# rasd3/3D-Dual-Fusion

Measured on AMD Instinct MI355X. Metric: nuScenes sweeps/sec (0.075 m voxel, ~60k pts), higher is better.
Workload: dtype f32 (fp32-grade throughout: every matrix-core GEMM -- C>=32 sparse convs, neck / head convs, FFN, query linears, image projection, value GEMM -- takes its fp32 operands as fp16 hi+lo pairs, 22 significand bits, 3 MFMA products, fp32 accumulate: <= 4e-6 of scale against float64, the grade of the exac

## Files before the change

3d-dual-fusion_amd/csrc/ffn.hip:

```cpp
#include <stdlib.h>

#include <string.h>

#include "common.h"

namespace df3d {

DF3D_SPLIT_OVERFLOW_TU(ffn)

constexpr int FFN_WQ = 8 * 2 * 64;

template <int C>
__global__ __launch_bounds__(256) void pack_ffn_kernel(const float *__restrict__ w1, const float *__restrict__ w2,
                                                       int H, u32x4 *__restrict__ out) {
  constexpr int KB = C / 32, CT = C / 16, SPC = KB + 4;
  size_t i = (size_t)blockIdx.x * blockDim.x + threadIdx.x;
  size_t total = (size_t)(H / 128) * SPC * FFN_WQ;
  if (i >= total) return;
  int lane = (int)(i & 63);
  int part = (int)((i >> 6) & 1);
  int t = (int)((i >> 7) & 7);
  int sj = (int)((i >> 10) % SPC);
  int c = (int)((i >> 10) / SPC);
  int n = lane & 15, g = lane >> 4;
  float wv[8];
#pragma unroll
  for (int e = 0; e < 8; ++e) {
    float w = 0.f;
    if (sj < KB) {
      int hid = c * 128 + t * 16 + n;
      int ch = sj * 32 + g * 8 + e;
      w = w1[(size_t)hid * C + ch];
    } else if (t < CT) {
      int q = sj - KB;
      int col = n * CT + t;
      int hid = c * 128 + (2 * q + (e >> 2)) * 16 + 4 * g + (e & 3);
      w = w2[(size_t)col * H + hid];
    }
    wv[e] = w;
  }
  u32x4 o;
#pragma unroll
  for (int e = 0; e < 4; ++e) {
    unsigned hi, lo;
    split_pair_w(wv[2 * e], wv[2 * e + 1], hi, lo);
    o[e] = part ? lo : hi;
  }
  out[i] = o;
}

struct FfnArgs {
  const float *x;
  const u32x4 *w;
  const float *b1, *b2;
  const float *res;
  const float *ln_g, *ln_b;
  float eps;
  float *out;
  long long rows;
  int H;
  int dbg;
  int bf16;
};

struct FfnJobs {
  FfnArgs s[4];
};

template <int NW, int RT, int NP = 2, int C = 128>
__global__ __launch_bounds__(NW * 64) void ffn_split_kernel(FfnJobs jobs) {
  constexpr int KB = C / 32, CT = C / 16, SPC = KB + 4;
  const FfnArgs &a = jobs.s[blockIdx.y];
  if ((long long)blockIdx.x * (16 * RT * NW) >= a.rows) return;
  constexpr int NT = NW * 64, WR = 16 * RT, TM = NW * WR;
  constexpr int WPT = FFN_WQ / NT;
  static_assert(FFN_WQ % NT == 0, "tile must divide over the workgroup");
  __shared__ u32x4 Wl[2][FFN_WQ];

  const int tid = threadIdx.x, lane = tid & 63, wave = tid >> 6;
  const int g = lane >> 4, n = lane & 15;
  const long long wrow0 = (long long)blockIdx.x * TM + wave * WR;
  const int nchunks = a.H / 128;
  const int steps = nchunks * SPC;

  u32x4 xh[RT][KB], xl[RT][KB];
#pragma unroll
  for (int rt = 0; rt < RT; ++rt) {
    const long long row_n = wrow0 + rt * 16 + n;
    const long long row_ld = row_n < a.rows ? row_n : a.rows - 1;
#pragma unroll
    for (int kb = 0; kb < KB; ++kb) {
      const float *p = a.x + row_ld * C + kb * 32 + g * 8;
      f32x4 v0 = *(const f32x4 *)p, v1 = *(const f32x4 *)(p + 4);
      split_pair(v0[0], v0[1], xh[rt][kb][0], xl[rt][kb][0]);
      split_pair(v0[2], v0[3], xh[rt][kb][1], xl[rt][kb][1]);
      split_pair(v1[0], v1[1], xh[rt][kb][2], xl[rt][kb][2]);
      split_pair(v1[2], v1[3], xh[rt][kb][3], xl[rt][kb][3]);
    }
  }

  static_assert(SPC % 2 == 0, "register set = step parity");
  u32x4 wreg[2][WPT];
  auto load_w = [&](int s, int set) {
    s = s < steps ? s : steps - 1;
    const u32x4 *src = a.w + (size_t)s * FFN_WQ;
#pragma unroll
    for (int i = 0; i < WPT; ++i) wreg[set][i] = src[tid + NT * i];
  };
  auto store_w = [&](int buf, int set) {
#pragma unroll
    for (int i = 0; i < WPT; ++i) Wl[buf][tid + NT * i] = wreg[set][i];
  };

  f32x4 acc2[RT][CT];
#pragma unroll
  for (int rt = 0; rt < RT; ++rt)
#pragma unroll
    for (int ct = 0; ct < CT; ++ct) acc2[rt][ct] = (f32x4){0.f, 0.f, 0.f, 0.f};

  load_w(0, 0);
  store_w(0, 0);
  load_w(1, 1);
  load_w(2, 0);
  for (int c = 0; c < nchunks; ++c) {
    f32x4 acc1[RT][8];
#pragma unroll
    for (int rt = 0; rt < RT; ++rt)
#pragma unroll
      for (int t = 0; t < 8; ++t) acc1[rt][t] = (f32x4){0.f, 0.f, 0.f, 0.f};
#pragma unroll
    for (int kb = 0; kb < KB; ++kb) {
      const int s = c * SPC + kb;
      __syncthreads();
      if (!(a.dbg & 2)) {
        store_w((s + 1) & 1, (kb + 1) & 1);
        load_w(s + 3, (kb + 1) & 1);
      }
      const u32x4 *wb = Wl[s & 1] + lane;
      if (a.dbg & 1) continue;
      u32x4 fq[2][4];
#pragma unroll
      for (int q = 0; q < 4; q += (NP == 2 ? 1 : 2)) fq[0][q] = wb[q * 64];
#pragma unroll
      for (int t = 0; t < 8; t += 2) {
        const int cur = (t >> 1) & 1;
        if (t + 2 < 8) {
#pragma unroll
          for (int q = 0; q < 4; q += (NP == 2 ? 1 : 2)) fq[cur ^ 1][q] = wb[((t + 2) * 2 + q) * 64];
        }
        const u32x4 ah0 = fq[cur][0], al0 = fq[cur][1], ah1 = fq[cur][2], al1 = fq[cur][3];
        if constexpr (NP == 2) {
#pragma unroll
          for (int rt = 0; rt < RT; ++rt) {
            acc1[rt][t] = DF3D_MFMA_F16(ah0, xl[rt][kb], acc1[rt][t]);
            acc1[rt][t + 1] = DF3D_MFMA_F16(ah1, xl[rt][kb], acc1[rt][t + 1]);
          }
#pragma unroll
          for (int rt = 0; rt < RT; ++rt) {
            acc1[rt][t] = DF3D_MFMA_F16(al0, xh[rt][kb], acc1[rt][t]);
            acc1[rt][t + 1] = DF3D_MFMA_F16(al1, xh[rt][kb], acc1[rt][t + 1]);
          }
        }
#pragma unroll
        for (int rt = 0; rt < RT; ++rt) {
          acc1[rt][t] = DF3D_MFMA_F16(ah0, xh[rt][kb], acc1[rt][t]);
          acc1[rt][t + 1] = DF3D_MFMA_F16(ah1, xh[rt][kb], acc1[rt][t + 1]);
        }
      }
    }
    u32x4 hh[RT][4], hl[RT][4];
#pragma unroll
    for (int q = 0; q < 4; ++q) {
#pragma unroll
      for (int half = 0; half < 2; ++half) {
        const int t = 2 * q + half;
        const f32x4 b = *(const f32x4 *)(a.b1 + c * 128 + t * 16 + 4 * g);
#pragma unroll
        for (int rt = 0; rt < RT; ++rt) {
          const f32x4 hv = acc1[rt][t] * DF3D_ACC_UNSCALE + b;
          split_pair_nc(fmaxf(hv[0], 0.f), fmaxf(hv[1], 0.f), hh[rt][q][half * 2], hl[rt][q][half * 2]);
          split_pair_nc(fmaxf(hv[2], 0.f), fmaxf(hv[3], 0.f), hh[rt][q][half * 2 + 1], hl[rt][q][half * 2 + 1]);
        }
      }
    }
#pragma unroll
    for (int q = 0; q < 4; ++q) {
      const int s = c * SPC + KB + q;
      __syncthreads();
      if (!(a.dbg & 2)) {
        store_w((s + 1) & 1, (KB + q + 1) & 1);
        load_w(s + 3, (KB + q + 1) & 1);
      }
      const u32x4 *wb = Wl[s & 1] + lane;
      if (a.dbg & 1) continue;
      u32x4 fq[2][4];
#pragma unroll
      for (int k = 0; k < 4; k += (NP == 2 ? 1 : 2)) fq[0][k] = wb[k * 64];
#pragma unroll
      for (int ct = 0; ct < CT; ct += 2) {
        const int cur = (ct >> 1) & 1;
        if (ct + 2 < CT) {
#pragma unroll
          for (int k = 0; k < 4; k += (NP == 2 ? 1 : 2)) fq[cur ^ 1][k] = wb[((ct + 2) * 2 + k) * 64];
        }
        const u32x4 bh0 = fq[cur][0], bl0 = fq[cur][1], bh1 = fq[cur][2], bl1 = fq[cur][3];
        if constexpr (NP == 2) {
#pragma unroll
          for (int rt = 0; rt < RT; ++rt) {
            acc2[rt][ct] = DF3D_MFMA_F16(hl[rt][q], bh0, acc2[rt][ct]);
            acc2[rt][ct + 1] = DF3D_MFMA_F16(hl[rt][q], bh1, acc2[rt][ct + 1]);
          }
#pragma unroll
          for (int rt = 0; rt < RT; ++rt) {
            acc2[rt][ct] = DF3D_MFMA_F16(hh[rt][q], bl0, acc2[rt][ct]);
            acc2[rt][ct + 1] = DF3D_MFMA_F16(hh[rt][q], bl1, acc2[rt][ct + 1]);
          }
        }
#pragma unroll
        for (int rt = 0; rt < RT; ++rt) {
          acc2[rt][ct] = DF3D_MFMA_F16(hh[rt][q], bh0, acc2[rt][ct]);
          acc2[rt][ct + 1] = DF3D_MFMA_F16(hh[rt][q], bh1, acc2[rt][ct + 1]);
        }
      }
    }
  }

  constexpr int NV = CT / 4;
  f32x4 bias[NV], gam[NV], bet[NV];
#pragma unroll
  for (int v = 0; v < NV; ++v) {
    bias[v] = *(const f32x4 *)(a.b2 + n * CT + 4 * v);
    gam[v] = (f32x4){1.f, 1.f, 1.f, 1.f};
    bet[v] = (f32x4){0.f, 0.f, 0.f, 0.f};
    if (a.ln_g) {
      gam[v] = *(const f32x4 *)(a.ln_g + n * CT + 4 * v);
      bet[v] = *(const f32x4 *)(a.ln_b + n * CT + 4 * v);
    }
  }
#pragma unroll
  for (int rt = 0; rt < RT; ++rt) {
    const long long rbase = wrow0 + rt * 16 + 4 * g;
#pragma unroll
    for (int r = 0; r < 4; ++r) {
      const long long row = rbase + r;
      const bool live = row < a.rows;
      const long long rr = live ? row : a.rows - 1;
      f32x4 val[NV];
      float s = 0.f;
#pragma unroll
      for (int v = 0; v < NV; ++v) {
        val[v] = (f32x4){acc2[rt][4 * v][r], acc2[rt][4 * v + 1][r], acc2[rt][4 * v + 2][r], acc2[rt][4 * v + 3][r]} *
                     DF3D_ACC_UNSCALE + bias[v];
        if (a.res) val[v] += *(const f32x4 *)(a.res + rr * C + n * CT + 4 * v);
        s += val[v][0] + val[v][1] + val[v][2] + val[v][3];
      }
      if (a.ln_g) {
#pragma unroll
        for (int o = 8; o >= 1; o >>= 1) s += __shfl_xor(s, o, 64);
        const float mean = s * (1.f / C);
        float ss = 0.f;
#pragma unroll
        for (int v = 0; v < NV; ++v) {
          val[v] = val[v] - mean;
          ss += val[v][0] * val[v][0] + val[v][1] * val[v][1] + val[v][2] * val[v][2] + val[v][3] * val[v][3];
        }
#pragma unroll
        for (int o = 8; o >= 1; o >>= 1) ss += __shfl_xor(ss, o, 64);
        const float rstd = rsqrtf(ss * (1.f / C) + a.eps);
#pragma unroll
        for (int v = 0; v < NV; ++v) val[v] = val[v] * rstd * gam[v] + bet[v];
      }
      if (live) {
#pragma unroll
        for (int v = 0; v < NV; ++v) *(f32x4 *)(a.out + row * C + n * CT + 4 * v) = val[v];
      }
    }
  }
}

}

using namespace df3d;

extern "C" size_t df3d_ffn_packed_bytes(int d_model, int d_ffn) {
  if ((d_model != 128 && d_model != 64) || d_ffn <= 0 || d_ffn % 128 != 0) return 0;
  return (size_t)(d_ffn / 128) * (d_model / 32 + 4) * FFN_WQ * 16;
}

extern "C" int df3d_ffn_pack(const float *w1, const float *w2, int d_model, int d_ffn, void *packed, void *stream_) {
  hipStream_t stream = (hipStream_t)stream_;
  DF3D_CHECK_ARG(w1 && w2 && packed, "ffn_pack: null argument");
  DF3D_CHECK_ARG(df3d_ffn_packed_bytes(d_model, d_ffn) != 0,
                 "ffn_pack: the fused feed-forward kernel serves d_model 64 / 128 and d_ffn %% 128 == 0 (got %d, %d)",
                 d_model, d_ffn);
  size_t total = (size_t)(d_ffn / 128) * (d_model / 32 + 4) * FFN_WQ;
  if (d_model == 128)
    hipLaunchKernelGGL(pack_ffn_kernel<128>, dim3(cdiv((long long)total, 256)), dim3(256), 0, stream, w1, w2, d_ffn,
                       (u32x4 *)packed);
  else
    hipLaunchKernelGGL(pack_ffn_kernel<64>, dim3(cdiv((long long)total, 256)), dim3(256), 0, stream, w1, w2, d_ffn,
                       (u32x4 *)packed);
  DF3D_LAUNCH_CHECK();
  return DF3D_OK;
}

static int ffn_launch(const FfnJobs &jobs, int njobs, long long max_rows, int d_model, hipStream_t stream) {
  if (d_model == 64) {
    static const int cfg64 = getenv("DF3D_FFN_CFG64") ? atoi(getenv("DF3D_FFN_CFG64")) : 0;
    if (!jobs.s[0].bf16 && cfg64 == 44) {
      hipLaunchKernelGGL((ffn_split_kernel<4, 4, 2, 64>), dim3(cdiv(max_rows, 256), njobs), dim3(256), 0, stream, jobs);
      DF3D_LAUNCH_CHECK();
      return DF3D_OK;
    }
    if (!jobs.s[0].bf16 && (cfg64 == 82 || (cfg64 == 0 && (long long)cdiv(max_rows, 256) * njobs >= 192))) {
      hipLaunchKernelGGL((ffn_split_kernel<8, 2, 2, 64>), dim3(cdiv(max_rows, 256), njobs), dim3(512), 0, stream, jobs);
      DF3D_LAUNCH_CHECK();
      return DF3D_OK;
    }
    if (jobs.s[0].bf16)
      hipLaunchKernelGGL((ffn_split_kernel<8, 1, 1, 64>), dim3(cdiv(max_rows, 128), njobs), dim3(512), 0, stream, jobs);
    else
      hipLaunchKernelGGL((ffn_split_kernel<8, 1, 2, 64>), dim3(cdiv(max_rows, 128), njobs), dim3(512), 0, stream, jobs);
    DF3D_LAUNCH_CHECK();
    return DF3D_OK;
  }
  static const int cfg_env = getenv("DF3D_FFN_CFG") ? atoi(getenv("DF3D_FFN_CFG")) : 0;
  static int ncu = 0;
  if (!ncu) {
    hipDeviceProp_t prop;
    ncu = (hipGetDeviceProperties(&prop, 0) == hipSuccess && prop.multiProcessorCount > 0) ? prop.multiProcessorCount : 256;
  }
  const long long wg82 = (long long)cdiv(max_rows, 256) * njobs;
  static const bool balance = !(getenv("DF3D_FFN_PAD") && getenv("DF3D_FFN_PAD")[0] == '0');
  const int cfg = cfg_env ? cfg_env : (wg82 >= 160 && !(balance && wg82 > ncu) ? 82 : 81);
  if (jobs.s[0].bf16) {
    if (max_rows >= 32 * 1024 && cfg != 81 + 1000)
      hipLaunchKernelGGL((ffn_split_kernel<8, 2, 1>), dim3(cdiv(max_rows, 256), njobs), dim3(512), 0, stream, jobs);
    else
      hipLaunchKernelGGL((ffn_split_kernel<8, 1, 1>), dim3(cdiv(max_rows, 128), njobs), dim3(512), 0, stream, jobs);
    DF3D_LAUNCH_CHECK();
    return DF3D_OK;
  }
  if (cfg == 44) hipLaunchKernelGGL((ffn_split_kernel<4, 4>), dim3(cdiv(max_rows, 256), njobs), dim3(256), 0, stream, jobs);
  else if (cfg == 42) hipLaunchKernelGGL((ffn_split_kernel<4, 2>), dim3(cdiv(max_rows, 128), njobs), dim3(256), 0, stream, jobs);
  else if (cfg == 82) {
    size_t pad = 0;
    if (balance && wg82 <= ncu) {
      pad = 52 * 1024;
      static bool attr = false;
      if (!attr) {
        attr = hipFuncSetAttribute((const void *)ffn_split_kernel<8, 2>, hipFuncAttributeMaxDynamicSharedMemorySize,
                                   (int)pad) == hipSuccess;
        if (!attr) pad = 0;
      }
    }
    hipLaunchKernelGGL((ffn_split_kernel<8, 2>), dim3(cdiv(max_rows, 256), njobs), dim3(512), pad, stream, jobs);
  }
  else if (cfg == 41) hipLaunchKernelGGL((ffn_split_kernel<4, 1>), dim3(cdiv(max_rows, 64), njobs), dim3(256), 0, stream, jobs);
  else hipLaunchKernelGGL((ffn_split_kernel<8, 1>), dim3(cdiv(max_rows, 128), njobs), dim3(512), 0, stream, jobs);
  DF3D_LAUNCH_CHECK();
  return DF3D_OK;
}

static int g_ffn_bf16 = 0;
extern "C" int df3d_ffn_set_precision(int bf16) {
  g_ffn_bf16 = bf16 ? 1 : 0;
  return DF3D_OK;
}

extern "C" int df3d_ffn_fused(const float *x, long long rows, int d_model, int d_ffn, const void *packed,
                              const float *b1, const float *b2, const float *residual, const float *ln_weight,
                              const float *ln_bias, float eps, float *out, void *stream_) {
  hipStream_t stream = (hipStream_t)stream_;
  DF3D_CHECK_ARG(x && packed && b1 && b2 && out, "ffn_fused: null argument");
  DF3D_CHECK_ARG(df3d_ffn_packed_bytes(d_model, d_ffn) != 0, "ffn_fused: unsupported sizes d_model=%d d_ffn=%d",
                 d_model, d_ffn);
  DF3D_CHECK_ARG((ln_weight == nullptr) == (ln_bias == nullptr), "ffn_fused: LayerNorm needs weight and bias");
  if (rows <= 0) return DF3D_OK;
  FfnJobs jobs;
  memset(&jobs, 0, sizeof(jobs));
  jobs.s[0] = {x, (const u32x4 *)packed, b1, b2, residual, ln_weight, ln_bias, eps, out, rows, d_ffn,
               getenv("DF3D_FFN_DBG") ? atoi(getenv("DF3D_FFN_DBG")) : 0, g_ffn_bf16};
  return ffn_launch(jobs, 1, rows, d_model, stream);
}

extern "C" int df3d_ffn_fused_jobs(const df3d_ffn_job *j, int njobs, int d_model, int d_ffn, void *stream_) {
  hipStream_t stream = (hipStream_t)stream_;
  DF3D_CHECK_ARG(j && njobs >= 1 && njobs <= 4, "ffn_fused_jobs: 1..4 jobs");
  DF3D_CHECK_ARG(df3d_ffn_packed_bytes(d_model, d_ffn) != 0, "ffn_fused_jobs: unsupported sizes d_model=%d d_ffn=%d",
                 d_model, d_ffn);
  FfnJobs jobs;
  memset(&jobs, 0, sizeof(jobs));
  long long max_rows = 0;
  static const int dbg = getenv("DF3D_FFN_DBG") ? atoi(getenv("DF3D_FFN_DBG")) : 0;
  for (int i = 0; i < njobs; ++i) {
    DF3D_CHECK_ARG(j[i].rows <= 0 || (j[i].x && j[i].packed && j[i].b1 && j[i].b2 && j[i].out),
                   "ffn_fused_jobs: job %d has a null argument", i);
    DF3D_CHECK_ARG((j[i].ln_weight == nullptr) == (j[i].ln_bias == nullptr),
                   "ffn_fused_jobs: LayerNorm needs weight and bias");
    jobs.s[i] = {j[i].x, (const u32x4 *)j[i].packed, j[i].b1, j[i].b2, j[i].residual, j[i].ln_weight, j[i].ln_bias,
                 j[i].eps, j[i].out, j[i].rows > 0 ? j[i].rows : 0, d_ffn, dbg, g_ffn_bf16};
    if (j[i].rows > max_rows) max_rows = j[i].rows;
  }
  if (max_rows <= 0) return DF3D_OK;
  return ffn_launch(jobs, njobs, max_rows, d_model, stream);
}
```

Baseline: 404.0.

## Restructure fused FFN into 32-wide hidden stages with lagged ReLU/split overlap

Repacks FFN weights so each pipeline stage holds a 32-wide hidden slice of both W1 and W2, and rewrites the kernel to stream these stages through dynamic LDS. For RT>=2 it uses three buffers and a one-stage lag, so the bias+ReLU+hi/lo split of the previous slice is interleaved between the current slice's first-GEMM MFMAs, with scheduling barriers pinning the placement. This targets the serial epilogue bubble between the two GEMMs and cuts hidden-activation register pressure. In exchange it costs more LDS per workgroup, which can lower occupancy. It also drops the debug flag, the LDS padding balance heuristic and the 44 configs.

```diff
diff --git a/3d-dual-fusion_amd/csrc/ffn.hip b/3d-dual-fusion_amd/csrc/ffn.hip
--- a/3d-dual-fusion_amd/csrc/ffn.hip
+++ b/3d-dual-fusion_amd/csrc/ffn.hip
@@ -2,43 +2,50 @@
 
 #include <string.h>
 
+#include <type_traits>
+
 #include "common.h"
 
 namespace df3d {
 
 DF3D_SPLIT_OVERFLOW_TU(ffn)
 
-constexpr int FFN_WQ = 8 * 2 * 64;
+template <int C>
+struct FfnStage {
+  static constexpr int KB = C / 32, CT = C / 16;
+  static constexpr int W2O = KB * 4 * 64;
+  static constexpr int STQ = (KB * 4 + CT * 2) * 64;
+};
 
 template <int C>
 __global__ __launch_bounds__(256) void pack_ffn_kernel(const float *__restrict__ w1, const float *__restrict__ w2,
                                                        int H, u32x4 *__restrict__ out) {
-  constexpr int KB = C / 32, CT = C / 16, SPC = KB + 4;
+  constexpr int KB = C / 32, CT = C / 16, FPS = FfnStage<C>::STQ / 64;
   size_t i = (size_t)blockIdx.x * blockDim.x + threadIdx.x;
-  size_t total = (size_t)(H / 128) * SPC * FFN_WQ;
+  size_t total = (size_t)(H / 32) * FfnStage<C>::STQ;
   if (i >= total) return;
   int lane = (int)(i & 63);
-  int part = (int)((i >> 6) & 1);
-  int t = (int)((i >> 7) & 7);
-  int sj = (int)((i >> 10) % SPC);
-  int c = (int)((i >> 10) / SPC);
+  int f = (int)((i >> 6) % FPS);
+  int Q = (int)((i >> 6) / FPS);
+  int c = Q >> 2, q = Q & 3;
   int n = lane & 15, g = lane >> 4;
+  int part;
   float wv[8];
 #pragma unroll
   for (int e = 0; e < 8; ++e) {
-    float w = 0.f;
-    if (sj < KB) {
-      int hid = c * 128 + t * 16 + n;
-      int ch = sj * 32 + g * 8 + e;
-      w = w1[(size_t)hid * C + ch];
-    } else if (t < CT) {
-      int q = sj - KB;
-      int col = n * CT + t;
+    if (f < KB * 4) {
+      int half = (f >> 1) & 1, kb = f >> 2;
+      int hid = c * 128 + (2 * q + half) * 16 + n;
+      int ch = kb * 32 + g * 8 + e;
+      wv[e] = w1[(size_t)hid * C + ch];
+    } else {
+      int ct = (f - KB * 4) >> 1;
+      int col = n * CT + ct;
       int hid = c * 128 + (2 * q + (e >> 2)) * 16 + 4 * g + (e & 3);
-      w = w2[(size_t)col * H + hid];
-    }
-    wv[e] = w;
-  }
+      wv[e] = w2[(size_t)col * H + hid];
+    }
+  }
+  part = f & 1;
   u32x4 o;
 #pragma unroll
   for (int e = 0; e < 4; ++e) {
@@ -59,7 +66,6 @@
   float *out;
   long long rows;
   int H;
-  int dbg;
   int bf16;
 };
 
@@ -67,21 +73,30 @@
   FfnArgs s[4];
 };
 
+template <int RT, int C>
+constexpr size_t ffn_lds_bytes() {
+  return (size_t)(RT >= 2 ? 3 : 2) * FfnStage<C>::STQ * 16;
+}
+
 template <int NW, int RT, int NP = 2, int C = 128>
 __global__ __launch_bounds__(NW * 64) void ffn_split_kernel(FfnJobs jobs) {
-  constexpr int KB = C / 32, CT = C / 16, SPC = KB + 4;
+  constexpr int KB = C / 32, CT = C / 16, STQ = FfnStage<C>::STQ, W2O = FfnStage<C>::W2O;
+  constexpr bool LAG = RT >= 2;
+  constexpr int NB = LAG ? 3 : 2;
   const FfnArgs &a = jobs.s[blockIdx.y];
   if ((long long)blockIdx.x * (16 * RT * NW) >= a.rows) return;
   constexpr int NT = NW * 64, WR = 16 * RT, TM = NW * WR;
-  constexpr int WPT = FFN_WQ / NT;
-  static_assert(FFN_WQ % NT == 0, "tile must divide over the workgroup");
-  __shared__ u32x4 Wl[2][FFN_WQ];
-
+  constexpr int WPT = STQ / NT;
+  static_assert(STQ % NT == 0, "stage must divide over the workgroup");
+  extern __shared__ u32x4 Wl[];
+
+  const int NS = a.H / 32;
+  const int wave_s = __builtin_amdgcn_readfirstlane(threadIdx.x >> 6);
+  f32x4 acc2[RT][CT];
+  {
   const int tid = threadIdx.x, lane = tid & 63, wave = tid >> 6;
   const int g = lane >> 4, n = lane & 15;
   const long long wrow0 = (long long)blockIdx.x * TM + wave * WR;
-  const int nchunks = a.H / 128;
-  const int steps = nchunks * SPC;
 
   u32x4 xh[RT][KB], xl[RT][KB];
 #pragma unroll
@@ -99,132 +114,165 @@
     }
   }
 
-  static_assert(SPC % 2 == 0, "register set = step parity");
-  u32x4 wreg[2][WPT];
-  auto load_w = [&](int s, int set) {
-    s = s < steps ? s : steps - 1;
-    const u32x4 *src = a.w + (size_t)s * FFN_WQ;
-#pragma unroll
-    for (int i = 0; i < WPT; ++i) wreg[set][i] = src[tid + NT * i];
+  u32x4 wreg[WPT];
+  auto load_w = [&](int s) {
+    s = s < NS ? s : NS - 1;
+    const u32x4 *src = a.w + (size_t)s * STQ;
+#pragma unroll
+    for (int i = 0; i < WPT; ++i) wreg[i] = src[tid + NT * i];
   };
-  auto store_w = [&](int buf, int set) {
-#pragma unroll
-    for (int i = 0; i < WPT; ++i) Wl[buf][tid + NT * i] = wreg[set][i];
+  auto store_w = [&](int buf) {
+#pragma unroll
+    for (int i = 0; i < WPT; ++i) Wl[buf * STQ + tid + NT * i] = wreg[i];
   };
-
-  f32x4 acc2[RT][CT];
+  f32x4 bq[2];
+  auto load_b = [&](int Q) {
+    Q = Q < NS ? Q : NS - 1;
+#pragma unroll
+    for (int half = 0; half < 2; ++half) bq[half] = *(const f32x4 *)(a.b1 + Q * 32 + half * 16 + 4 * g);
+  };
+
 #pragma unroll
   for (int rt = 0; rt < RT; ++rt)
 #pragma unroll
     for (int ct = 0; ct < CT; ++ct) acc2[rt][ct] = (f32x4){0.f, 0.f, 0.f, 0.f};
-
-  load_w(0, 0);
-  store_w(0, 0);
-  load_w(1, 1);
-  load_w(2, 0);
-  for (int c = 0; c < nchunks; ++c) {
-    f32x4 acc1[RT][8];
-#pragma unroll
-    for (int rt = 0; rt < RT; ++rt)
-#pragma unroll
-      for (int t = 0; t < 8; ++t) acc1[rt][t] = (f32x4){0.f, 0.f, 0.f, 0.f};
-#pragma unroll
-    for (int kb = 0; kb < KB; ++kb) {
-      const int s = c * SPC + kb;
-      __syncthreads();
-      if (!(a.dbg & 2)) {
-        store_w((s + 1) & 1, (kb + 1) & 1);
-        load_w(s + 3, (kb + 1) & 1);
-      }
-      const u32x4 *wb = Wl[s & 1] + lane;
-      if (a.dbg & 1) continue;
+  u32x4 hh[RT], hl[RT];
+
+  auto split_piece = [&](const f32x4(&src)[RT][2], int hp) {
+    const int rt = hp >> 2, half = (hp >> 1) & 1, sub = hp & 1;
+    const float h0 = src[rt][half][2 * sub] * DF3D_ACC_UNSCALE + bq[half][2 * sub];
+    const float h1 = src[rt][half][2 * sub + 1] * DF3D_ACC_UNSCALE + bq[half][2 * sub + 1];
+    split_pair_nc(fmaxf(h0, 0.f), fmaxf(h1, 0.f), hh[rt][half * 2 + sub], hl[rt][half * 2 + sub]);
+  };
+  auto pin = [&]() { __builtin_amdgcn_sched_barrier(0x4 | 0x10 | 0x80); };
+
+  auto stage = [&](int S, int bcur, int bprev, int bnext, f32x4(&cur)[RT][2], f32x4(&prev)[RT][2], auto P1, auto P2,
+                   auto ST) {
+    constexpr bool p1 = decltype(P1)::value, p2 = decltype(P2)::value;
+    constexpr int NHP = RT * 4;
+    constexpr bool ride = LAG && p1 && p2;
+    __syncthreads();
+    __builtin_amdgcn_sched_barrier(0);
+    if constexpr (decltype(ST)::value) {
+      store_w(bnext);
+      load_w(S + 2);
+    }
+    if constexpr (p1) {
+      const u32x4 *wb = Wl + bcur * STQ + lane;
+#pragma unroll
+      for (int rt = 0; rt < RT; ++rt) cur[rt][0] = cur[rt][1] = (f32x4){0.f, 0.f, 0.f, 0.f};
       u32x4 fq[2][4];
 #pragma unroll
-      for (int q = 0; q < 4; q += (NP == 2 ? 1 : 2)) fq[0][q] = wb[q * 64];
-#pragma unroll
-      for (int t = 0; t < 8; t += 2) {
-        const int cur = (t >> 1) & 1;
-        if (t + 2 < 8) {
-#pragma unroll
-          for (int q = 0; q < 4; q += (NP == 2 ? 1 : 2)) fq[cur ^ 1][q] = wb[((t + 2) * 2 + q) * 64];
-        }
-        const u32x4 ah0 = fq[cur][0], al0 = fq[cur][1], ah1 = fq[cur][2], al1 = fq[cur][3];
+      for (int k = 0; k < 4; k += (NP == 2 ? 1 : 2)) fq[0][k] = wb[k * 64];
+#pragma unroll
+      for (int kb = 0; kb < KB; ++kb) {
+        const int cb = kb & 1;
+        if (kb + 1 < KB) {
+#pragma unroll
+          for (int k = 0; k < 4; k += (NP == 2 ? 1 : 2)) fq[cb ^ 1][k] = wb[((kb + 1) * 4 + k) * 64];
+        }
+        const u32x4 ah0 = fq[cb][0], al0 = fq[cb][1], ah1 = fq[cb][2], al1 = fq[cb][3];
+        const int hp0 = kb * NHP / KB, hp2 = (kb + 1) * NHP / KB, hp1 = (hp0 + hp2) / 2;
         if constexpr (NP == 2) {
 #pragma unroll
           for (int rt = 0; rt < RT; ++rt) {
-            acc1[rt][t] = DF3D_MFMA_F16(ah0, xl[rt][kb], acc1[rt][t]);
-            acc1[rt][t + 1] = DF3D_MFMA_F16(ah1, xl[rt][kb], acc1[rt][t + 1]);
+            cur[rt][0] = DF3D_MFMA_F16(ah0, xl[rt][kb], cur[rt][0]);
+            cur[rt][1] = DF3D_MFMA_F16(ah1, xl[rt][kb], cur[rt][1]);
           }
+        }
+        if constexpr (ride) {
+          pin();
+#pragma unroll
+          for (int hp = hp0; hp < hp1; ++hp) split_piece(prev, hp);
+          pin();
+        }
+        if constexpr (NP == 2) {
 #pragma unroll
           for (int rt = 0; rt < RT; ++rt) {
-            acc1[rt][t] = DF3D_MFMA_F16(al0, xh[rt][kb], acc1[rt][t]);
-            acc1[rt][t + 1] = DF3D_MFMA_F16(al1, xh[rt][kb], acc1[rt][t + 1]);
+            cur[rt][0] = DF3D_MFMA_F16(al0, xh[rt][kb], cur[rt][0]);
+            cur[rt][1] = DF3D_MFMA_F16(al1, xh[rt][kb], cur[rt][1]);
           }
         }
+        if constexpr (ride) {
+          pin();
+#pragma unroll
+          for (int hp = hp1; hp < hp2; ++hp) split_piece(prev, hp);
+          pin();
+        }
 #pragma unroll
         for (int rt = 0; rt < RT; ++rt) {
-          acc1[rt][t] = DF3D_MFMA_F16(ah0, xh[rt][kb], acc1[rt][t]);
-          acc1[rt][t + 1] = DF3D_MFMA_F16(ah1, xh[rt][kb], acc1[rt][t + 1]);
-        }
-      }
-    }
-    u32x4 hh[RT][4], hl[RT][4];
-#pragma unroll
-    for (int q = 0; q < 4; ++q) {
-#pragma unroll
-      for (int half = 0; half < 2; ++half) {
-        const int t = 2 * q + half;
-        const f32x4 b = *(const f32x4 *)(a.b1 + c * 128 + t * 16 + 4 * g);
+          cur[rt][0] = DF3D_MFMA_F16(ah0, xh[rt][kb], cur[rt][0]);
+          cur[rt][1] = DF3D_MFMA_F16(ah1, xh[rt][kb], cur[rt][1]);
+        }
+      }
+    }
+    if constexpr (p2) {
+      if constexpr (!ride) {
+#pragma unroll
+        for (int hp = 0; hp < NHP; ++hp) split_piece(LAG ? prev : cur, hp);
+      }
+      if constexpr (ride) pin();
+      load_b(LAG ? S : S + 1);
+      const u32x4 *wb2 = Wl + (LAG ? bprev : bcur) * STQ + W2O + lane;
+      u32x4 f2[2][4];
+#pragma unroll
+      for (int k = 0; k < 4; k += (NP == 2 ? 1 : 2)) f2[0][k] = wb2[k * 64];
+#pragma unroll
+      for (int ct = 0; ct < CT; ct += 2) {
+        const int cb = (ct >> 1) & 1;
+        if (ct + 2 < CT) {
+#pragma unroll
+          for (int k = 0; k < 4; k += (NP == 2 ? 1 : 2)) f2[cb ^ 1][k] = wb2[((ct + 2) * 2 + k) * 64];
+        }
+        const u32x4 bh0 = f2[cb][0], bl0 = f2[cb][1], bh1 = f2[cb][2], bl1 = f2[cb][3];
+        if constexpr (NP == 2) {
+#pragma unroll
+          for (int rt = 0; rt < RT; ++rt) {
+            acc2[rt][ct] = DF3D_MFMA_F16(hl[rt], bh0, acc2[rt][ct]);
+            acc2[rt][ct + 1] = DF3D_MFMA_F16(hl[rt], bh1, acc2[rt][ct + 1]);
+          }
+#pragma unroll
+          for (int rt = 0; rt < RT; ++rt) {
+            acc2[rt][ct] = DF3D_MFMA_F16(hh[rt], bl0, acc2[rt][ct]);
+            acc2[rt][ct + 1] = DF3D_MFMA_F16(hh[rt], bl1, acc2[rt][ct + 1]);
+          }
+        }
 #pragma unroll
         for (int rt = 0; rt < RT; ++rt) {
-          const f32x4 hv = acc1[rt][t] * DF3D_ACC_UNSCALE + b;
-          split_pair_nc(fmaxf(hv[0], 0.f), fmaxf(hv[1], 0.f), hh[rt][q][half * 2], hl[rt][q][half * 2]);
-          split_pair_nc(fmaxf(hv[2], 0.f), fmaxf(hv[3], 0.f), hh[rt][q][half * 2 + 1], hl[rt][q][half * 2 + 1]);
-        }
-      }
-    }
-#pragma unroll
-    for (int q = 0; q < 4; ++q) {
-      const int s = c * SPC + KB + q;
-      __syncthreads();
-      if (!(a.dbg & 2)) {
-        store_w((s + 1) & 1, (KB + q + 1) & 1);
-        load_w(s + 3, (KB + q + 1) & 1);
-      }
-      const u32x4 *wb = Wl[s & 1] + lane;
-      if (a.dbg & 1) continue;
-      u32x4 fq[2][4];
-#pragma unroll
-      for (int k = 0; k < 4; k += (NP == 2 ? 1 : 2)) fq[0][k] = wb[k * 64];
-#pragma unroll
-      for (int ct = 0; ct < CT; ct += 2) {
-        const int cur = (ct >> 1) & 1;
-        if (ct + 2 < CT) {
-#pragma unroll
-          for (int k = 0; k < 4; k += (NP == 2 ? 1 : 2)) fq[cur ^ 1][k] = wb[((ct + 2) * 2 + k) * 64];
-        }
-        const u32x4 bh0 = fq[cur][0], bl0 = fq[cur][1], bh1 = fq[cur][2], bl1 = fq[cur][3];
-        if constexpr (NP == 2) {
-#pragma unroll
-          for (int rt = 0; rt < RT; ++rt) {
-            acc2[rt][ct] = DF3D_MFMA_F16(hl[rt][q], bh0, acc2[rt][ct]);
-            acc2[rt][ct + 1] = DF3D_MFMA_F16(hl[rt][q], bh1, acc2[rt][ct + 1]);
-          }
-#pragma unroll
-          for (int rt = 0; rt < RT; ++rt) {
-            acc2[rt][ct] = DF3D_MFMA_F16(hh[rt][q], bl0, acc2[rt][ct]);
-            acc2[rt][ct + 1] = DF3D_MFMA_F16(hh[rt][q], bl1, acc2[rt][ct + 1]);
-          }
-        }
-#pragma unroll
-        for (int rt = 0; rt < RT; ++rt) {
-          acc2[rt][ct] = DF3D_MFMA_F16(hh[rt][q], bh0, acc2[rt][ct]);
-          acc2[rt][ct + 1] = DF3D_MFMA_F16(hh[rt][q], bh1, acc2[rt][ct + 1]);
-        }
-      }
-    }
-  }
-
+          acc2[rt][ct] = DF3D_MFMA_F16(hh[rt], bh0, acc2[rt][ct]);
+          acc2[rt][ct + 1] = DF3D_MFMA_F16(hh[rt], bh1, acc2[rt][ct + 1]);
+        }
+      }
+    }
+  };
+
+  constexpr std::true_type yes{};
+  constexpr std::false_type no{};
+  f32x4 accA[RT][2], accB[RT][2];
+  load_w(0);
+  store_w(0);
+  load_w(1);
+  load_b(0);
+  if constexpr (LAG) {
+    stage(0, 0, 2, 1, accA, accB, yes, no, yes);
+    int b = 1;
+    for (int S = 1; S + 1 < NS; S += 2) {
+      const int b1 = b == 2 ? 0 : b + 1, b2 = b1 == 2 ? 0 : b1 + 1;
+      stage(S, b, b2, b1, accB, accA, yes, yes, yes);
+      stage(S + 1, b1, b, b2, accA, accB, yes, yes, yes);
+      b = b2;
+    }
+    const int b1 = b == 2 ? 0 : b + 1, b2 = b1 == 2 ? 0 : b1 + 1;
+    stage(NS - 1, b, b2, b1, accB, accA, yes, yes, no);
+    stage(NS, b1, b, b2, accA, accB, no, yes, no);
+  } else {
+    for (int S = 0; S < NS; ++S) stage(S, S & 1, 0, (S + 1) & 1, accA, accA, yes, yes, yes);
+  }
+  }
+
+  const int lane_e = __builtin_amdgcn_mbcnt_hi(~0u, __builtin_amdgcn_mbcnt_lo(~0u, 0u));
+  const int g = lane_e >> 4, n = lane_e & 15;
+  const long long wrow0 = (long long)blockIdx.x * TM + wave_s * WR;
   constexpr int NV = CT / 4;
   f32x4 bias[NV], gam[NV], bet[NV];
 #pragma unroll
@@ -284,7 +332,7 @@
 
 extern "C" size_t df3d_ffn_packed_bytes(int d_model, int d_ffn) {
   if ((d_model != 128 && d_model != 64) || d_ffn <= 0 || d_ffn % 128 != 0) return 0;
-  return (size_t)(d_ffn / 128) * (d_model / 32 + 4) * FFN_WQ * 16;
+  return (size_t)(d_ffn / 32) * (d_model == 128 ? FfnStage<128>::STQ : FfnStage<64>::STQ) * 16;
 }
 
 extern "C" int df3d_ffn_pack(const float *w1, const float *w2, int d_model, int d_ffn, void *packed, void *stream_) {
@@ -293,7 +341,7 @@
   DF3D_CHECK_ARG(df3d_ffn_packed_bytes(d_model, d_ffn) != 0,
                  "ffn_pack: the fused feed-forward kernel serves d_model 64 / 128 and d_ffn %% 128 == 0 (got %d, %d)",
                  d_model, d_ffn);
-  size_t total = (size_t)(d_ffn / 128) * (d_model / 32 + 4) * FFN_WQ;
+  size_t total = df3d_ffn_packed_bytes(d_model, d_ffn) / 16;
   if (d_model == 128)
     hipLaunchKernelGGL(pack_ffn_kernel<128>, dim3(cdiv((long long)total, 256)), dim3(256), 0, stream, w1, w2, d_ffn,
                        (u32x4 *)packed);
@@ -304,25 +352,25 @@
   return DF3D_OK;
 }
 
+template <int NW, int RT, int NP, int C>
+static int ffn_launch_as(const FfnJobs &jobs, int njobs, long long max_rows, hipStream_t stream) {
+  constexpr size_t lds = ffn_lds_bytes<RT, C>();
+  static const bool attr = hipFuncSetAttribute((const void *)ffn_split_kernel<NW, RT, NP, C>,
+                                               hipFuncAttributeMaxDynamicSharedMemorySize, (int)lds) == hipSuccess;
+  DF3D_CHECK_ARG(attr, "ffn_fused: the device refuses %d bytes of LDS per workgroup", (int)lds);
+  hipLaunchKernelGGL((ffn_split_kernel<NW, RT, NP, C>), dim3(cdiv(max_rows, NW * RT * 16), njobs), dim3(NW * 64), lds,
+                     stream, jobs);
+  DF3D_LAUNCH_CHECK();
+  return DF3D_OK;
+}
+
 static int ffn_launch(const FfnJobs &jobs, int njobs, long long max_rows, int d_model, hipStream_t stream) {
   if (d_model == 64) {
     static const int cfg64 = getenv("DF3D_FFN_CFG64") ? atoi(getenv("DF3D_FFN_CFG64")) : 0;
-    if (!jobs.s[0].bf16 && cfg64 == 44) {
-      hipLaunchKernelGGL((ffn_split_kernel<4, 4, 2, 64>), dim3(cdiv(max_rows, 256), njobs), dim3(256), 0, stream, jobs);
-      DF3D_LAUNCH_CHECK();
-      return DF3D_OK;
-    }
-    if (!jobs.s[0].bf16 && (cfg64 == 82 || (cfg64 == 0 && (long long)cdiv(max_rows, 256) * njobs >= 192))) {
-      hipLaunchKernelGGL((ffn_split_kernel<8, 2, 2, 64>), dim3(cdiv(max_rows, 256), njobs), dim3(512), 0, stream, jobs);
-      DF3D_LAUNCH_CHECK();
-      return DF3D_OK;
-    }
-    if (jobs.s[0].bf16)
-      hipLaunchKernelGGL((ffn_split_kernel<8, 1, 1, 64>), dim3(cdiv(max_rows, 128), njobs), dim3(512), 0, stream, jobs);
-    else
-      hipLaunchKernelGGL((ffn_split_kernel<8, 1, 2, 64>), dim3(cdiv(max_rows, 128), njobs), dim3(512), 0, stream, jobs);
-    DF3D_LAUNCH_CHECK();
-    return DF3D_OK;
+    if (jobs.s[0].bf16) return ffn_launch_as<8, 1, 1, 64>(jobs, njobs, max_rows, stream);
+    if (cfg64 == 82 || (cfg64 == 0 && (long long)cdiv(max_rows, 256) * njobs >= 192))
+      return ffn_launch_as<8, 2, 2, 64>(jobs, njobs, max_rows, stream);
+    return ffn_launch_as<8, 1, 2, 64>(jobs, njobs, max_rows, stream);
   }
   static const int cfg_env = getenv("DF3D_FFN_CFG") ? atoi(getenv("DF3D_FFN_CFG")) : 0;
   static int ncu = 0;
@@ -331,35 +379,15 @@
     ncu = (hipGetDeviceProperties(&prop, 0) == hipSuccess && prop.multiProcessorCount > 0) ? prop.multiProcessorCount : 256;
   }
   const long long wg82 = (long long)cdiv(max_rows, 256) * njobs;
-  static const bool balance = !(getenv("DF3D_FFN_PAD") && getenv("DF3D_FFN_PAD")[0] == '0');
-  const int cfg = cfg_env ? cfg_env : (wg82 >= 160 && !(balance && wg82 > ncu) ? 82 : 81);
+  const int cfg = cfg_env ? cfg_env : (wg82 >= 160 && wg82 <= ncu ? 82 : 81);
   if (jobs.s[0].bf16) {
-    if (max_rows >= 32 * 1024 && cfg != 81 + 1000)
-      hipLaunchKernelGGL((ffn_split_kernel<8, 2, 1>), dim3(cdiv(max_rows, 256), njobs), dim3(512), 0, stream, jobs);
-    else
-      hipLaunchKernelGGL((ffn_split_kernel<8, 1, 1>), dim3(cdiv(max_rows, 128), njobs), dim3(512), 0, stream, jobs);
-    DF3D_LAUNCH_CHECK();
-    return DF3D_OK;
-  }
-  if (cfg == 44) hipLaunchKernelGGL((ffn_split_kernel<4, 4>), dim3(cdiv(max_rows, 256), njobs), dim3(256), 0, stream, jobs);
-  else if (cfg == 42) hipLaunchKernelGGL((ffn_split_kernel<4, 2>), dim3(cdiv(max_rows, 128), njobs), dim3(256), 0, stream, jobs);
-  else if (cfg == 82) {
-    size_t pad = 0;
-    if (balance && wg82 <= ncu) {
-      pad = 52 * 1024;
-      static bool attr = false;
-      if (!attr) {
-        attr = hipFuncSetAttribute((const void *)ffn_split_kernel<8, 2>, hipFuncAttributeMaxDynamicSharedMemorySize,
-                                   (int)pad) == hipSuccess;
-        if (!attr) pad = 0;
-      }
-    }
-    hipLaunchKernelGGL((ffn_split_kernel<8, 2>), dim3(cdiv(max_rows, 256), njobs), dim3(512), pad, stream, jobs);
-  }
-  else if (cfg == 41) hipLaunchKernelGGL((ffn_split_kernel<4, 1>), dim3(cdiv(max_rows, 64), njobs), dim3(256), 0, stream, jobs);
-  else hipLaunchKernelGGL((ffn_split_kernel<8, 1>), dim3(cdiv(max_rows, 128), njobs), dim3(512), 0, stream, jobs);
-  DF3D_LAUNCH_CHECK();
-  return DF3D_OK;
+    if (max_rows >= 32 * 1024 && cfg != 81 + 1000) return ffn_launch_as<8, 2, 1, 128>(jobs, njobs, max_rows, stream);
+    return ffn_launch_as<8, 1, 1, 128>(jobs, njobs, max_rows, stream);
+  }
+  if (cfg == 42) return ffn_launch_as<4, 2, 2, 128>(jobs, njobs, max_rows, stream);
+  if (cfg == 82) return ffn_launch_as<8, 2, 2, 128>(jobs, njobs, max_rows, stream);
+  if (cfg == 41) return ffn_launch_as<4, 1, 2, 128>(jobs, njobs, max_rows, stream);
+  return ffn_launch_as<8, 1, 2, 128>(jobs, njobs, max_rows, stream);
 }
 
 static int g_ffn_bf16 = 0;
@@ -379,8 +407,7 @@
   if (rows <= 0) return DF3D_OK;
   FfnJobs jobs;
   memset(&jobs, 0, sizeof(jobs));
-  jobs.s[0] = {x, (const u32x4 *)packed, b1, b2, residual, ln_weight, ln_bias, eps, out, rows, d_ffn,
-               getenv("DF3D_FFN_DBG") ? atoi(getenv("DF3D_FFN_DBG")) : 0, g_ffn_bf16};
+  jobs.s[0] = {x, (const u32x4 *)packed, b1, b2, residual, ln_weight, ln_bias, eps, out, rows, d_ffn, g_ffn_bf16};
   return ffn_launch(jobs, 1, rows, d_model, stream);
 }
 
@@ -392,14 +419,13 @@
   FfnJobs jobs;
   memset(&jobs, 0, sizeof(jobs));
   long long max_rows = 0;
-  static const int dbg = getenv("DF3D_FFN_DBG") ? atoi(getenv("DF3D_FFN_DBG")) : 0;
   for (int i = 0; i < njobs; ++i) {
     DF3D_CHECK_ARG(j[i].rows <= 0 || (j[i].x && j[i].packed && j[i].b1 && j[i].b2 && j[i].out),
                    "ffn_fused_jobs: job %d has a null argument", i);
     DF3D_CHECK_ARG((j[i].ln_weight == nullptr) == (j[i].ln_bias == nullptr),
                    "ffn_fused_jobs: LayerNorm needs weight and bias");
     jobs.s[i] = {j[i].x, (const u32x4 *)j[i].packed, j[i].b1, j[i].b2, j[i].residual, j[i].ln_weight, j[i].ln_bias,
-                 j[i].eps, j[i].out, j[i].rows > 0 ? j[i].rows : 0, d_ffn, dbg, g_ffn_bf16};
+                 j[i].eps, j[i].out, j[i].rows > 0 ? j[i].rows : 0, d_ffn, g_ffn_bf16};
     if (j[i].rows > max_rows) max_rows = j[i].rows;
   }
   if (max_rows <= 0) return DF3D_OK;
```

New measurement: 409.9, median of 4. +1.5%, better.
